# Komputerowe-Projektowanie-Lekow/pmarlo

Hardware: AMD Instinct MI355X
Metric: frames/sec featurize->TICA->k-means->T-matrix, 1Mx64 synth; ITS rel-err (higher is better)
Workload: dtype f64; 1 GPU; synthetic 1000000 frames x 64 f32 features per GPU (AR(1) latents), TICA->10, k=500 (10 Lloyd iterations), lag=10, row-normalised T; frames_per_gpu=1000000, features=64, tica_dim=10, k=500, lag=10, kmeans_iters=10, parallelism=shards1

## Files before the change

### pmarlo_amd/csrc/eig.hip

```cpp
#include "common.h"
#include "wave.h"

__device__ __forceinline__ unsigned long long stamp_clock() {
    unsigned long long t;
    asm volatile("s_memtime %0\n\ts_waitcnt lgkmcnt(0)" : "=s"(t)::"memory");
    return t;
}
#define STAMP_ADD(slot, last) do { const unsigned long long t__ = stamp_clock(); slot += t__ - last; last = t__; } while (0)
#ifdef MSM_JACOBI_STAMPS
__device__ unsigned long long g_jacobi_stamps[8];
#define JSTAMP(i) STAMP_ADD(acc__[i], last__)
#define JSTAMP_INIT unsigned long long acc__[8] = {0, 0, 0, 0, 0, 0, 0, 0}; unsigned long long last__ = stamp_clock();
#define JSTAMP_FLUSH if (threadIdx.x == 0) { for (int i__ = 0; i__ < 8; ++i__) g_jacobi_stamps[i__] += acc__[i__]; }
#else
#define JSTAMP(i)
#define JSTAMP_INIT
#define JSTAMP_FLUSH
#endif
#ifdef MSM_TRI_STAMPS
__device__ unsigned long long g_tri_stamps[24];
#define TSTAMP(i) do { if (threadIdx.x == 0) STAMP_ADD(g_tri_stamps[i], tlast__); } while (0)
#define TSTAMP_INIT unsigned long long tlast__ = 0; if (threadIdx.x == 0) tlast__ = stamp_clock();
#define KSTAMP(i) do { if (threadIdx.x == 0) STAMP_ADD(g_tri_stamps[i], klast__); } while (0)
#define KSTAMP_INIT unsigned long long klast__ = 0; if (threadIdx.x == 0) klast__ = stamp_clock();
#else
#define TSTAMP(i)
#define TSTAMP_INIT
#define KSTAMP(i)
#define KSTAMP_INIT
#endif
#ifdef MSM_TRI_STAMPS_FINE
#define LSTAMP(i) TSTAMP(i)
#define LSTAMP_INIT TSTAMP_INIT
#else
#define LSTAMP(i)
#define LSTAMP_INIT
#endif

namespace {

constexpr int kEigThreads = 1024;
constexpr int kMaxPairs = 128;

struct JacobiShared {
    double2 cs[kMaxPairs];
    int p[kMaxPairs], q[kMaxPairs];
    int reserved[2 * kMaxPairs];
    double2 cs2[2][32];
    int colw2[2][32], roww2[2][32];
    double red[kEigThreads / 64];
    double bc[4];
    int ibc[4];
};

__device__ __forceinline__ double nr_rcp(double x) {
    double r = __builtin_amdgcn_rcp(x);
    r = fma(r, fma(-x, r, 1.0), r);
    r = fma(r, fma(-x, r, 1.0), r);
    return r;
}
__device__ __forceinline__ double nr_rsqrt(double x) {
    double r = __builtin_amdgcn_rsq(x);
    const double h = 0.5 * x;
    r = r * fma(-h * r, r, 1.5);
    r = r * fma(-h * r, r, 1.5);
    return r;
}

__device__ __forceinline__ void jacobi_rotation(double app, double aqq, double apq, double& c, double& s) {
    c = 1.0; s = 0.0;
    if (apq == 0.0) return;
    const double a = 0.5 * (aqq - app);
    const double h2 = fma(a, a, apq * apq);
    if (!(h2 > 1e-300) || !(h2 < 1e300)) return;
    double rh = __builtin_amdgcn_rsq(h2);
    rh = rh * fma(-0.5 * h2 * rh, rh, 1.5);
    const double h = h2 * rh;
    const double den = fabs(a) + h;
    double rd = __builtin_amdgcn_rcp(den);
    rd = fma(rd, fma(-den, rd, 1.0), rd);
    const double t = (a >= 0.0 ? apq : -apq) * rd;
    c = nr_rsqrt(fma(t, t, 1.0));
    s = t * c;
}

__device__ __forceinline__ void pivot_pair(int round, int i, int npad, int& p, int& q) {
    if (i == 0) { p = round; q = npad - 1; return; }
    p = round + i; if (p >= npad - 1) p -= npad - 1;
    q = round - i; if (q < 0) q += npad - 1;
}

__device__ __forceinline__ void rotate_pair(double c, double s, double& xp, double& xq) {
    const double yp = fma(-s, xq, c * xp), yq = fma(s, xp, c * xq);
    xp = yp; xq = yq;
}

__device__ __forceinline__ void rotate_block(double app, double apq, double aqp, double aqq, double ca, double sa,
                                             double cb, double sb, bool diagonal, double& npp, double& npq,
                                             double& nqp, double& nqq) {
    const double rpp = fma(-sa, aqp, ca * app), rpq = fma(-sa, aqq, ca * apq);
    const double rqp = fma(sa, app, ca * aqp), rqq = fma(sa, apq, ca * aqq);
    npp = fma(-sb, rpq, cb * rpp); npq = fma(sb, rpp, cb * rpq);
    nqp = fma(-sb, rqq, cb * rqp); nqq = fma(sb, rqp, cb * rqq);
    if (diagonal) { npq = 0.0; nqp = 0.0; }
}

__device__ __forceinline__ void set_identity(double* V, int n, int ld) {
    for (int i = threadIdx.x; i < n * n; i += blockDim.x) V[(i / n) * ld + (i % n)] = (i / n == i % n) ? 1.0 : 0.0;
}

__device__ __forceinline__ bool jacobi_converged(const double* A, int n, int ld, JacobiShared* sh) {
    double off = 0.0, dia = 0.0;
    for (int i = threadIdx.x; i < n * n; i += blockDim.x) {
        const int r = i / n, c = i - r * n;
        const double v = A[r * ld + c];
        if (r == c) dia = fma(v, v, dia); else off = fma(v, v, off);
    }
    off = block_sum_bcast(off, sh->red, sh->bc);
    dia = block_sum_bcast(dia, sh->red, sh->bc);
    const double tol = (double)n * 2.220446049250313e-16;
    return off <= tol * tol * (dia + off) || off == 0.0;
}

__device__ __forceinline__ int jacobi_eigh_pipelined(double* A, double* V, int n, int ld, JacobiShared* sh,
                                                     int max_sweeps);

__device__ __forceinline__ int jacobi_eigh(double* A, double* V, int n, int ld, JacobiShared* sh, int max_sweeps) {
    const int tid = threadIdx.x, nt = blockDim.x;
    {
        const int mh = n / 2;
        if ((n & 1) == 0 && mh >= 4 && mh <= 32 && mh * mh <= nt && mh * n <= 2 * nt && n * ld < 65536 && nt >= 64)
            return jacobi_eigh_pipelined(A, V, n, ld, sh, max_sweeps);
    }
    set_identity(V, n, ld);
    __syncthreads();
    if (n < 2) return 0;
    const int npad = n + (n & 1);
    const int m = npad / 2;
    int sweep = 0;
    JSTAMP_INIT
    for (; sweep < max_sweeps; ++sweep) {
        JSTAMP(0);
        if (jacobi_converged(A, n, ld, sh)) break;
        JSTAMP(1);
        const bool fast = (m * m <= nt) && (m * n <= 2 * nt);
        const int my_ia = tid / m, my_ib = tid - my_ia * m;
        const bool has_blk = tid < m * m;
        const int v_ib0 = tid / n, v_r0 = tid - v_ib0 * n;
        const int v_ib1 = (tid + nt) / n, v_r1 = (tid + nt) - v_ib1 * n;
        const bool has_v0 = tid < m * n, has_v1 = tid + nt < m * n;
        const int my_ia_c = has_blk ? my_ia : 0, my_ib_c = has_blk ? my_ib : 0;
        const int v_ib0_c = has_v0 ? v_ib0 : 0, v_ib1_c = has_v1 ? v_ib1 : 0;
        const int v_r1_c = has_v1 ? v_r1 : 0;
        for (int round = 0; round < npad - 1; ++round) {
            if (tid < m) {
                const int i = tid;
                int p, q;
                pivot_pair(round, i, npad, p, q);
                double c = 1.0, s = 0.0;
                if (q < n) jacobi_rotation(A[p * ld + p], A[q * ld + q], A[p * ld + q], c, s);
                sh->cs[i] = make_double2(c, s); sh->p[i] = p; sh->q[i] = q;
            }
            JSTAMP(2);
            __syncthreads();
            JSTAMP(3);
            if (fast) {
                int pa, qa, pb, qb, vp0, vq0, vp1, vq1;
                pivot_pair(round, my_ia_c, npad, pa, qa);
                pivot_pair(round, my_ib_c, npad, pb, qb);
                pivot_pair(round, v_ib0_c, npad, vp0, vq0);
                pivot_pair(round, v_ib1_c, npad, vp1, vq1);
                const bool row_real = qa < n, col_real = qb < n, v0 = has_v0 && vq0 < n, v1 = has_v1 && vq1 < n;
                const int qa_c = row_real ? qa : pa, qb_c = col_real ? qb : pb;
                const int vq0_c = vq0 < n ? vq0 : vp0, vq1_c = vq1 < n ? vq1 : vp1;
                const double2 ra = sh->cs[my_ia_c], rb = sh->cs[my_ib_c], r0 = sh->cs[v_ib0_c], r1 = sh->cs[v_ib1_c];
                const double app = A[pa * ld + pb], apq = A[pa * ld + qb_c];
                const double aqp = A[qa_c * ld + pb], aqq = A[qa_c * ld + qb_c];
                double x0p = V[v_r0 * ld + vp0], x0q = V[v_r0 * ld + vq0_c];
                double x1p = V[v_r1_c * ld + vp1], x1q = V[v_r1_c * ld + vq1_c];
                const double ca = row_real ? ra.x : 1.0, sa = row_real ? ra.y : 0.0;
                const double cb = col_real ? rb.x : 1.0, sb = col_real ? rb.y : 0.0;
                double npp, npq, nqp, nqq;
                rotate_block(app, apq, aqp, aqq, ca, sa, cb, sb, my_ia_c == my_ib_c, npp, npq, nqp, nqq);
                rotate_pair(r0.x, r0.y, x0p, x0q);
                rotate_pair(r1.x, r1.y, x1p, x1q);
                if (has_blk) A[pa * ld + pb] = npp;
                if (has_blk && col_real) A[pa * ld + qb] = npq;
                if (has_blk && row_real) A[qa * ld + pb] = nqp;
                if (has_blk && row_real && col_real) A[qa * ld + qb] = nqq;
                if (v0) { V[v_r0 * ld + vp0] = x0p; V[v_r0 * ld + vq0] = x0q; }
                if (v1) { V[v_r1_c * ld + vp1] = x1p; V[v_r1_c * ld + vq1] = x1q; }
                JSTAMP(4);
                JSTAMP(5);
            } else {
                for (int blk = tid; blk < m * m; blk += nt) {
                    const int ia = blk / m, ib = blk - ia * m;
                    const int pa = sh->p[ia], qa = sh->q[ia], pb = sh->p[ib], qb = sh->q[ib];
                    const bool row_real = qa < n, col_real = qb < n;
                    if (!row_real && !col_real) continue;
                    const double ca = sh->cs[ia].x, sa = sh->cs[ia].y, cb = sh->cs[ib].x, sb = sh->cs[ib].y;
                    if (!col_real) {
                        double ap = A[pa * ld + pb], aq = A[qa * ld + pb];
                        rotate_pair(ca, sa, ap, aq);
                        A[pa * ld + pb] = ap; A[qa * ld + pb] = aq;
                        continue;
                    }
                    if (!row_real) {
                        double ap = A[pa * ld + pb], aq = A[pa * ld + qb];
                        rotate_pair(cb, sb, ap, aq);
                        A[pa * ld + pb] = ap; A[pa * ld + qb] = aq;
                        continue;
                    }
                    const double app = A[pa * ld + pb], apq = A[pa * ld + qb];
                    const double aqp = A[qa * ld + pb], aqq = A[qa * ld + qb];
                    double npp, npq, nqp, nqq;
                    rotate_block(app, apq, aqp, aqq, ca, sa, cb, sb, ia == ib, npp, npq, nqp, nqq);
                    A[pa * ld + pb] = npp; A[pa * ld + qb] = npq;
                    A[qa * ld + pb] = nqp; A[qa * ld + qb] = nqq;
                }
                JSTAMP(4);
                for (int e = tid; e < m * n; e += nt) {
                    const int ib = e / n, r = e - ib * n;
                    const int pb = sh->p[ib], qb = sh->q[ib];
                    if (qb >= n) continue;
                    const double cb = sh->cs[ib].x, sb = sh->cs[ib].y;
                    double vp = V[r * ld + pb], vq = V[r * ld + qb];
                    rotate_pair(cb, sb, vp, vq);
                    V[r * ld + pb] = vp; V[r * ld + qb] = vq;
                }
                JSTAMP(5);
            }
            __syncthreads();
            JSTAMP(6);
        }
    }
    JSTAMP_FLUSH
    return sweep;
}

__device__ __forceinline__ int jacobi_eigh_pipelined(double* A, double* V, int n, int ld, JacobiShared* sh,
                                                     int max_sweeps) {
    const int tid = threadIdx.x, nt = blockDim.x;
    set_identity(V, n, ld);
    const int m = n / 2, ring = n - 1;
    auto form_rotations = [&](int round, int buf) {
        int p, q;
        pivot_pair(round, tid, n, p, q);
        double c, s;
        jacobi_rotation(A[p * ld + p], A[q * ld + q], A[p * ld + q], c, s);
        sh->cs2[buf][tid] = make_double2(c, s);
        sh->colw2[buf][tid] = p | (q << 16);
        sh->roww2[buf][tid] = (p * ld) | ((q * ld) << 16);
    };
    auto update_block = [&](int ia, int ib, int buf, bool live) {
        const int wr = sh->roww2[buf][ia], wc = sh->colw2[buf][ib];
        const double2 ra = sh->cs2[buf][ia], rb = sh->cs2[buf][ib];
        double* Ap = A + (wr & 0xffff);
        double* Aq = A + (wr >> 16);
        const int pb = wc & 0xffff, qb = wc >> 16;
        const double app = Ap[pb], apq = Ap[qb], aqp = Aq[pb], aqq = Aq[qb];
        double npp, npq, nqp, nqq;
        rotate_block(app, apq, aqp, aqq, ra.x, ra.y, rb.x, rb.y, ia == ib, npp, npq, nqp, nqq);
        if (live) { Ap[pb] = npp; Ap[qb] = npq; Aq[pb] = nqp; Aq[qb] = nqq; }
    };
    const int my_ia = tid / m, my_ib = tid - my_ia * m;
    const bool priority = (my_ib == my_ia) || (my_ia >= 2 && my_ib == my_ia - 2) || (my_ia == 1 && my_ib == 0) ||
                          (my_ia == m - 1 && my_ib == m - 2);
    const bool has_blk = tid < m * m && !priority;
    const int my_ia_c = tid < m * m ? my_ia : 0, my_ib_c = tid < m * m ? my_ib : 0;
    int pr_ia = 0, pr_ib = 0;
    const bool has_pr = tid < 2 * m;
    if (tid < m) { pr_ia = tid; pr_ib = tid; }
    else if (tid < 2 * m) {
        const int j = tid - m;
        if (j == 0) { pr_ia = 1; pr_ib = 0; }
        else if (j == 1) { pr_ia = 2; pr_ib = 0; }
        else if (j == m - 1) { pr_ia = m - 1; pr_ib = m - 2; }
        else { pr_ia = j + 1; pr_ib = j - 1; }
    }
    const int v_ib0 = tid / n, v_r0 = tid - v_ib0 * n;
    const int v_ib1 = (tid + nt) / n, v_r1 = (tid + nt) - v_ib1 * n;
    const bool has_v0 = tid < m * n, has_v1 = tid + nt < m * n;
    const int v_ib0_c = has_v0 ? v_ib0 : 0, v_ib1_c = has_v1 ? v_ib1 : 0, v_r1_c = has_v1 ? v_r1 : 0;
    __syncthreads();
    int buf = 0, round = 0;
    if (tid < m) form_rotations(0, 0);
    __syncthreads();
    int sweep = 0;
    for (; sweep < max_sweeps; ++sweep) {
        if (jacobi_converged(A, n, ld, sh)) break;
        for (int rr = 0; rr < ring; ++rr) {
            const int next_round = round + 1 == ring ? 0 : round + 1;
            if (tid < 64) {
                update_block(pr_ia, pr_ib, buf, has_pr);
                if (tid < m) form_rotations(next_round, buf ^ 1);
            }
            update_block(my_ia_c, my_ib_c, buf, has_blk);
            {
                const int w0 = sh->colw2[buf][v_ib0_c], w1 = sh->colw2[buf][v_ib1_c];
                const double2 r0 = sh->cs2[buf][v_ib0_c], r1 = sh->cs2[buf][v_ib1_c];
                double* V0 = V + v_r0 * ld;
                double* V1 = V + v_r1_c * ld;
                const int vp0 = w0 & 0xffff, vq0 = w0 >> 16, vp1 = w1 & 0xffff, vq1 = w1 >> 16;
                double x0p = V0[vp0], x0q = V0[vq0], x1p = V1[vp1], x1q = V1[vq1];
                rotate_pair(r0.x, r0.y, x0p, x0q);
                rotate_pair(r1.x, r1.y, x1p, x1q);
                if (has_v0) { V0[vp0] = x0p; V0[vq0] = x0q; }
                if (has_v1) { V1[vp1] = x1p; V1[vq1] = x1q; }
            }
            __syncthreads();
            buf ^= 1;
            round = next_round;
        }
    }
    return sweep;
}

__device__ void sort_desc_abs(const double* ev, int n, int* order) {
    rank_order<true>(n, order, [&](int i) { return fabs(ev[i]); });
    __syncthreads();
}

__device__ void canonical_signs(double* M, int n, int ncols, int ld) {
    for (int j = threadIdx.x; j < ncols; j += blockDim.x) {
        double best = -1.0, sgn = 1.0;
        for (int i = 0; i < n; ++i) {
            const double v = M[i * ld + j];
            if (fabs(v) > best) { best = fabs(v); sgn = v < 0.0 ? -1.0 : 1.0; }
        }
        if (sgn < 0.0)
            for (int i = 0; i < n; ++i) M[i * ld + j] = -M[i * ld + j];
    }
    __syncthreads();
}

__device__ bool cholesky_lower_pair(double* Mp, double* Mq, int n, int ld, JacobiShared* sh) {
    const int tid = threadIdx.x, nt = blockDim.x;
    for (int j = 0; j < n; ++j) {
        if (tid < 2) {
            double* M = tid == 0 ? Mp : Mq;
            const double dj = M[j * ld + j];
            sh->ibc[1 + tid] = dj > 0.0 ? 1 : 0;
            if (dj > 0.0) M[j * ld + j] = sqrt(dj);
        }
        __syncthreads();
        if (!sh->ibc[1] || !sh->ibc[2]) return false;
        const double pjj = Mp[j * ld + j], qjj = Mq[j * ld + j];
        for (int i = j + 1 + tid; i < n; i += nt) {
            Mp[i * ld + j] /= pjj;
            Mq[i * ld + j] /= qjj;
        }
        __syncthreads();
        const int m = n - j - 1;
        for (int e = tid; e < m * m; e += nt) {
            const int a = e / m, b = e - a * m;
            if (b <= a) {
                const int ra = (j + 1 + a) * ld, rb = (j + 1 + b) * ld;
                Mp[ra + j + 1 + b] -= Mp[ra + j] * Mp[rb + j];
                Mq[ra + j + 1 + b] -= Mq[ra + j] * Mq[rb + j];
            }
        }
        __syncthreads();
    }
    return true;
}

__device__ void lower_inverse(const double* G, double* X, int n, int ld) {
    const int tid = threadIdx.x, nt = blockDim.x;
    for (int e = tid; e < n * n; e += nt) {
        const int i = e / n, c = e - i * n;
        X[i * ld + c] = i == c ? 1.0 : 0.0;
    }
    __syncthreads();
    for (int k = 0; k < n; ++k) {
        const double gkk = G[k * ld + k];
        for (int c = tid; c <= k; c += nt) X[k * ld + c] /= gkk;
        __syncthreads();
        const int rows = n - k - 1, cols = k + 1;
        for (int e = tid; e < rows * cols; e += nt) {
            const int a = e / cols, c = e - a * cols;
            const int i = k + 1 + a;
            X[i * ld + c] = fma(-G[i * ld + k], X[k * ld + c], X[i * ld + c]);
        }
        __syncthreads();
    }
}

constexpr int kTriMax = 64;
constexpr int kTriLd = 65;
struct TriShared {
    double2 de[kTriMax + 8];
    double d[kTriMax], e[kTriMax], lam[kTriMax], praw[kTriMax], uq[kTriMax], inv[kTriMax];
    double scale, gl, gu;
    double red[kEigThreads / 64];
    int bad;
    double part[16][kTriMax];
    union {
        double2 vw[8][kTriMax];
        alignas(16) double lv[16][kTriMax];
    };
    double vpub[2][kTriMax];
    double taupub[2];
};

template <bool TA, bool TB>
__device__ __forceinline__ void mfma_mm(double* C, const double* A, const double* B, int rows, int cols, int inner, int ld,
                        const double* bscale = nullptr) {
    const int lane = threadIdx.x & 63, wave = threadIdx.x >> 6, nw = blockDim.x >> 6;
    const int j = lane & 15, g = lane >> 4;
    const int tr = (rows + 15) >> 4, tc = (cols + 15) >> 4;
    for (int t = wave; t < tr * tc; t += nw) {
        const int i0 = (t / tc) * 16, c0 = (t - (t / tc) * tc) * 16;
        const bool aok = i0 + j < rows, bok = c0 + j < cols;
        const int ai = aok ? i0 + j : 0, bj = bok ? c0 + j : 0;
        const double bs = bscale ? bscale[bj] : 1.0;
        const v4f64 acc = mfma_tile_acc(
            inner, g, aok, bok, [&](int k) { return TA ? A[k * ld + ai] : A[ai * ld + k]; },
            [&](int k) { return (TB ? B[bj * ld + k] : B[k * ld + bj]) * bs; });
#pragma unroll
        for (int r = 0; r < 4; ++r) {
            const int row = i0 + g + 4 * r, col = c0 + j;
            if (row < rows && col < cols) C[row * ld + col] = acc[r];
        }
    }
    __syncthreads();
}

__device__ __forceinline__ int sturm_count(const TriShared* ts, int nblocks, double x) {
    double pp = 0.0, p = 1.0;
    unsigned bits = 0, w0 = 0;
    for (int b = 0; b < nblocks; ++b) {
        asm volatile("" ::: "memory");
        double2 r[8];
#pragma unroll
        for (int u = 0; u < 8; ++u) r[u] = ts->de[8 * b + u];
#pragma unroll
        for (int u = 0; u < 8; ++u) {
            const double pn = fma(r[u].x - x, p, -(r[u].y * pp));
            bits = __builtin_amdgcn_alignbit(bits, (unsigned)__double2hiint(pn), 31);
            pp = p;
            p = pn;
        }
        if (b & 1) {
            const int ex = max(__builtin_amdgcn_frexp_exp(p), __builtin_amdgcn_frexp_exp(pp));
            p = ldexp(p, -ex);
            pp = ldexp(pp, -ex);
        }
        if (b == 3) { w0 = bits; bits = 0; }
    }
    if (nblocks <= 4) return __popc(bits ^ (bits >> 1));
    const int r1 = 8 * nblocks - 32;
    return __popc(w0 ^ (w0 >> 1)) + __popc(bits ^ ((bits >> 1) | ((w0 & 1u) << (r1 - 1))));
}

template <typename F>
__device__ __forceinline__ void hh_for_groups(int sub, int k, F&& body) {
#pragma unroll
    for (int g = 0; g < 2; ++g)
        if (sub + 32 * g + 24 > k) body(g);
}
__device__ __forceinline__ void householder_phase(double* A, double* QT, int n, TriShared* ts) {
    static_assert(kEigThreads == 1024, "householder_phase deals the rows of A and Q' over sixteen waves");
    constexpr int ld = kTriLd;
    const int lane = threadIdx.x & 63, wave = __builtin_amdgcn_readfirstlane(threadIdx.x >> 6);
    const bool in = lane < n;
    const bool is_a = wave < 8;
#ifdef MSM_TRI_NOQ
    const bool is_q = false;
#else
    const bool is_q = !is_a;
#endif
    const int sub = wave & 7;
    double* part = ts->part[wave];
    const double* parts = ts->part[is_a ? 0 : 8];
    double2* vw = ts->vw[sub];
    double m[8];
#pragma unroll
    for (int t = 0; t < 8; ++t) {
        const int j = sub + 8 * t;
        m[t] = (in && j < n) ? (is_a ? A[j * ld + lane] : (j == lane ? 1.0 : 0.0)) : 0.0;
    }
    auto q_partial = [&](int c) {
        if (__builtin_amdgcn_readfirstlane(ts->taupub[c & 1] != 0.0)) {
            const double* vp = ts->vpub[c & 1];
            double s0 = 0.0, s1 = 0.0;
            hh_for_groups(sub, c, [&](int g) {
                double v[4];
#pragma unroll
                for (int u = 0; u < 4; ++u) v[u] = vp[sub + 32 * g + 8 * u];
                s0 = fma(m[4 * g], v[0], s0);
                s1 = fma(m[4 * g + 1], v[1], s1);
                s0 = fma(m[4 * g + 2], v[2], s0);
                s1 = fma(m[4 * g + 3], v[3], s1);
            });
            part[lane] = s0 + s1;
        }
    };
    auto sum_parts = [&]() {
        return (((parts[lane] + parts[kTriMax + lane]) + (parts[2 * kTriMax + lane] + parts[3 * kTriMax + lane])) +
                ((parts[4 * kTriMax + lane] + parts[5 * kTriMax + lane]) + (parts[6 * kTriMax + lane] + parts[7 * kTriMax + lane])));
    };
    auto q_finish = [&](int c) {
        const double tau_c = ts->taupub[c & 1];
        if (__builtin_amdgcn_readfirstlane(tau_c != 0.0)) {
            const double* vp = ts->vpub[c & 1];
            const double tu = -tau_c * sum_parts();
            hh_for_groups(sub, c, [&](int g) {
                double v[4];
#pragma unroll
                for (int u = 0; u < 4; ++u) v[u] = vp[sub + 32 * g + 8 * u];
#pragma unroll
                for (int u = 0; u < 4; ++u) m[4 * g + u] = fma(tu, v[u], m[4 * g + u]);
            });
        }
    };
    auto reflector = [&](int c, double& vi, double& tau) {
        const double* rowc = A + c * ld;
        double xi = rowc[in ? lane : 0];
        const double alpha = rowc[c + 1];
        if (wave == 0 && lane == c) ts->d[c] = xi;
        const bool actc = in && lane > c;
        if (!actc) xi = 0.0;
        const double sigma = wave_sum_all(lane > c + 1 ? xi * xi : 0.0);
        const bool nz = sigma != 0.0;
        const double h2 = fma(alpha, alpha, sigma);
        const double rs = nr_rsqrt(nz ? h2 : 1.0);
        const double beta = nz ? -copysign(h2 * rs, alpha) : alpha;
        tau = nz ? (beta - alpha) * -copysign(rs, alpha) : 0.0;
        const double scal = nr_rcp(nz ? alpha - beta : 1.0);
        vi = actc ? (lane == c + 1 ? 1.0 : (nz ? xi * scal : 0.0)) : 0.0;
        if (wave == 0) {
            ts->vpub[c & 1][lane] = vi;
            if (lane == 0) { ts->e[c] = beta; ts->taupub[c & 1] = tau; }
        }
        vw[lane].x = vi;
    };
    LSTAMP_INIT
    double vi = 0.0, tau = 0.0;
    if (is_a && n > 2) reflector(0, vi, tau);
    for (int k = 0; k + 2 < n; ++k) {
        LSTAMP(16);
        const bool act = in && lane > k;
        if (is_a) {
            double s0 = 0.0, s1 = 0.0;
            hh_for_groups(sub, k, [&](int g) {
                double v[4];
#pragma unroll
                for (int u = 0; u < 4; ++u) v[u] = vw[sub + 32 * g + 8 * u].x;
                s0 = fma(m[4 * g], v[0], s0);
                s1 = fma(m[4 * g + 1], v[1], s1);
                s0 = fma(m[4 * g + 2], v[2], s0);
                s1 = fma(m[4 * g + 3], v[3], s1);
            });
            part[lane] = s0 + s1;
            LSTAMP(18);
        } else if (is_q && k > 0) {
            q_finish(k - 1);
        }
        __syncthreads();
        LSTAMP(19);
        double wi = 0.0;
        if (is_a) {
            const double p = sum_parts();
            const double pv = wave_sum_all(act ? p * vi : 0.0);
            const double al = -0.5 * tau * (tau * pv);
            wi = act ? fma(tau, p, al * vi) : 0.0;
            vw[lane].y = wi;
            LSTAMP(20);
#pragma unroll
            for (int t2 = 0; t2 < 8; ++t2)
                if (sub + 8 * t2 == k + 1) {
                    const double2 bk = vw[k + 1];
                    if (in) A[(k + 1) * ld + lane] = fma(-wi, bk.x, fma(-vi, bk.y, m[t2]));
                }
        } else if (is_q) {
            q_partial(k);
        }
        LSTAMP(21);
        __syncthreads();
        if (is_a) {
            double2 bb[8];
#pragma unroll
            for (int t2 = 0; t2 < 8; ++t2) bb[t2] = vw[sub + 8 * t2];
            const double vk = vi, wk = wi;
            if (k + 3 < n) reflector(k + 1, vi, tau);
#pragma unroll
            for (int t2 = 0; t2 < 8; ++t2) m[t2] = fma(-wk, bb[t2].x, fma(-vk, bb[t2].y, m[t2]));
            LSTAMP(17);
        }
    }
    if (is_q && n > 2) q_finish(n - 3);
    if (is_q && in) {
#pragma unroll
        for (int t = 0; t < 8; ++t)
            if (sub + 8 * t < n) QT[(sub + 8 * t) * ld + lane] = m[t];
    }
    if (is_a && in) {
#pragma unroll
        for (int t = 0; t < 8; ++t)
            if (sub + 8 * t >= n - 2 && sub + 8 * t < n) A[(sub + 8 * t) * ld + lane] = m[t];
    }
    __syncthreads();
    if (threadIdx.x == 0) {
        ts->d[n - 2] = A[(n - 2) * ld + n - 2];
        ts->e[n - 2] = A[(n - 1) * ld + n - 2];
        ts->d[n - 1] = A[(n - 1) * ld + n - 1];
        ts->e[n - 1] = 0.0;
    }
}

__device__ __forceinline__ bool ldl_whiten_registers(const double* C, double* W, int n, double epsilon, TriShared* ts,
                                                     int mode) {
    static_assert(kEigThreads == 1024, "ldl_whiten_registers deals the rows over sixteen waves");
    constexpr int ld = kTriLd;
    const int lane = threadIdx.x & 63, wave = __builtin_amdgcn_readfirstlane(threadIdx.x >> 6);
    const bool in = lane < n;
    const int what = mode == 2 ? (wave < 8 ? 2 : 3) : (wave < 8 ? 0 : 1);
    const int src = mode == 2 ? 2 : 0;
    const int sub = wave & 7;
    double m[8];
#pragma unroll
    for (int t = 0; t < 8; ++t) {
        const int i = sub + 8 * t;
        if (what == 1) m[t] = lane == i ? 1.0 : 0.0;
        else m[t] = (what < 3 && in && i < n) ? C[i * ld + lane] - (what == 2 && lane == i ? epsilon : 0.0) : 0.0;
    }
    if (sub == 0 && what < 3) ts->part[what][lane] = m[0];
    __syncthreads();
    LSTAMP_INIT
    for (int j = 0; j < n; ++j) {
        const int par = (j & 1) * 4;
        if (what < 3) {
            const double rowM = ts->part[par + src][lane];
            const double row = what == 1 ? ts->part[par + 1][lane] : rowM;
            const double d = readlane_f64(rowM, j);
            LSTAMP(13);
            if (!(d > 0.0)) return false;
            {
                const double lvec = lane > j ? rowM * nr_rcp(d) : 0.0;
                double* lv = ts->lv[wave];
                lv[(lane & 7) * 8 + (lane >> 3)] = lvec;
                const double2* mine = reinterpret_cast<const double2*>(lv + sub * 8);
#pragma unroll
                for (int t2 = 0; t2 < 4; ++t2) {
                    const double2 l = mine[t2];
                    m[2 * t2] = fma(-l.x, row, m[2 * t2]);
                    m[2 * t2 + 1] = fma(-l.y, row, m[2 * t2 + 1]);
                }
                if (((j + 1 - sub) & 7) == 0) {
                    double* dst = ts->part[(par ^ 4) + what] + lane;
                    switch ((j + 1 - sub) >> 3) {
                        case 0: *dst = m[0]; break;   case 1: *dst = m[1]; break;   case 2: *dst = m[2]; break;
                        case 3: *dst = m[3]; break;   case 4: *dst = m[4]; break;   case 5: *dst = m[5]; break;
                        case 6: *dst = m[6]; break;   case 7: *dst = m[7]; break;   default: break;
                    }
                }
            }
        } else {
            const double dP = ts->part[par + src][j];
            if (!(dP > 0.0)) return false;
        }
        LSTAMP(14);
        __syncthreads();
        LSTAMP(15);
    }
    if (what == 0) {
#pragma unroll
        for (int t = 0; t < 8; ++t)
            if (lane == sub + 8 * t && lane < n) ts->inv[lane] = nr_rsqrt(m[t]);
    }
    __syncthreads();
    if (what == 1 && in) {
#pragma unroll
        for (int t = 0; t < 8; ++t) {
            const int i = sub + 8 * t;
            if (i < n) W[lane * ld + i] = m[t] * ts->inv[i];
        }
    }
    __syncthreads();
    return true;
}

constexpr double kTriGuard = 1e-6;
__device__ __forceinline__ bool tridiag_eigh(double* A, double* Q, double* X, int n, int ld, TriShared* ts, double orth_tol,
                                             int want, int* sel, int& kept) {
    const int tid = threadIdx.x, nt = blockDim.x, lane = tid & 63, wave = tid >> 6;
    kept = 0;
    if (n == 1) {
        if (tid == 0) { ts->lam[0] = A[0]; A[0] = 1.0; }
        __syncthreads();
        return true;
    }
    if (ld != kTriLd) return false;
    TSTAMP_INIT
    if (tid == 0) ts->bad = 0;
    __syncthreads();
    TSTAMP(0);
    householder_phase(A, Q, n, ts);
    TSTAMP(1);
    __syncthreads();
    TSTAMP(2);
    {
        const double dl = lane < n ? ts->d[lane] : 0.0, el = lane < n ? ts->e[lane] : 0.0;
        double an = fmax(fabs(dl), fabs(el));
#pragma unroll
        for (int off = 32; off > 0; off >>= 1) an = fmax(an, __shfl_xor(an, off, 64));
        double sc = 1.0;
        if (an > 0.0 && an < 1e300) { int ex; (void)frexp(an, &ex); sc = ldexp(1.0, -ex); }
        const double ds = dl * sc, es = el * sc;
        const double em = lane > 0 && lane < n ? ts->e[lane - 1] * sc : 0.0;
        const double rad = fabs(em) + (lane + 1 < n ? fabs(es) : 0.0);
        double gl = lane < n ? ds - rad : 1e300, gu = lane < n ? ds + rad : -1e300;
        wave_minmax_xor(gl, gu);
        __syncthreads();
        if (wave == 0) {
            if (lane < n) { ts->d[lane] = ds; ts->e[lane] = es; ts->de[lane] = make_double2(ds, em * em); }
            else ts->de[lane] = make_double2(8.0, 0.0);
            if (lane < 8) ts->de[kTriMax + lane] = make_double2(8.0, 0.0);
            if (lane == 0) {
                if (!(an < 1e300)) ts->bad = 1;
                ts->scale = sc;
                const double bn = fmax(fabs(gl), fabs(gu));
                const double pad = 4.0 * n * 2.220446049250313e-16 * bn + 1e-290;
                ts->gl = gl - pad;
                ts->gu = gu + pad;
            }
        }
    }
    __syncthreads();
    TSTAMP(3);
    if (ts->bad) return false;
    bool lead = want > 0 && 2 * (want + 2) < n;
    int nb = lead ? 2 * (want + 2) : n;
    int na = n;
    for (;;) {
        if (tid < 8 * kTriMax && wave * 8 < nb) {
            const int b = tid >> 3, t = tid & 7;
            const int i = !lead || b < want + 2 ? b : n - nb + b;
            const int nblocks = (n + 7) >> 3;
            double lo = ts->gl, hi = ts->gu;
            const double frac = (double)(t + 1) * (1.0 / 9.0);
            for (int it = 0; it < 20; ++it) {
                const double x = fma(hi - lo, frac, lo);
                const int c = sturm_count(ts, nblocks, x);
                double nlo = c <= i ? x : lo, nhi = c > i ? x : hi;
                lo = row8_reduce(nlo, hw_max_f64);
                hi = row8_reduce(nhi, hw_min_f64);
            }
            if (b < nb && t == 0) ts->lam[i] = 0.5 * (lo + hi);
        }
        __syncthreads();
        if (!lead) break;
        const int nc = 2 * (want + 1);
        const auto cand = [&](int c) { return c <= want ? c : n - nc + c; };
        const auto key = [&](int c) { return fabs(ts->lam[cand(c)] / ts->scale); };
        rank_order<true>(nc, sel, key);
        __syncthreads();
        const bool lone = ts->lam[want + 1] - ts->lam[want] > kTriGuard &&
                          ts->lam[n - want - 1] - ts->lam[n - want - 2] > kTriGuard;
        if (lone && key(sel[want - 1]) != key(sel[want])) {
            const double lk = tid < nc ? ts->lam[cand(tid)] : 0.0;
            __syncthreads();
            if (tid < nc) ts->lam[tid] = lk;
            __syncthreads();
            na = nc;
            break;
        }
        __syncthreads();
        lead = false;
        nb = n;
    }
    TSTAMP(4);
    const double tiny = 1e-290;
    double* Xc = X + (lane < na ? lane : 0);
    double* Ac = A + (lane < na ? lane : 0);
    const double lamb = ts->lam[lane < na ? lane : 0];
    if (wave == 0 && lane < na) {
        double q = ts->de[0].x - lamb;
        Xc[0] = q;
        for (int j0 = 1; j0 < n; j0 += 8) {
            double2 r[8];
#pragma unroll
            for (int u = 0; u < 8; ++u) r[u] = ts->de[j0 + u];
#pragma unroll
            for (int u = 0; u < 8; ++u) {
                if (j0 + u < n) {
                    if (fabs(q) < tiny) q = -tiny;
                    q = fma(-r[u].y, nr_rcp(q), r[u].x - lamb);
                    Xc[(j0 + u) * ld] = q;
                }
            }
        }
    } else if (wave == 1 && lane < na) {
        double r = ts->de[n - 1].x - lamb;
        if (fabs(r) < tiny) r = -tiny;
        double ir = nr_rcp(r);
        Ac[(n - 1) * ld] = ir;
        for (int j0 = n - 2; j0 >= 0; j0 -= 8) {
            double dj[8], e2[8];
#pragma unroll
            for (int u = 0; u < 8; ++u) {
                const int j = j0 - u >= 0 ? j0 - u : 0;
                dj[u] = ts->de[j].x;
                e2[u] = ts->de[j + 1].y;
            }
#pragma unroll
            for (int u = 0; u < 8; ++u) {
                if (j0 - u >= 0) {
                    r = fma(-e2[u], ir, dj[u] - lamb);
                    if (fabs(r) < tiny) r = -tiny;
                    ir = nr_rcp(r);
                    Ac[(j0 - u) * ld] = ir;
                }
            }
        }
    }
    __syncthreads();
    int kk = n - 1;
    if (wave < 2 && lane < na) {
        double gbest = fabs(Xc[(n - 1) * ld]);
        for (int j0 = n - 2; j0 >= 0; j0 -= 8) {
            double g[8];
#pragma unroll
            for (int u = 0; u < 8; ++u) {
                const int j = j0 - u >= 0 ? j0 - u : 0;
                g[u] = fabs(fma(-ts->de[j + 1].y, Ac[(j + 1) * ld], Xc[j * ld]));
            }
#pragma unroll
            for (int u = 0; u < 8; ++u)
                if (j0 - u >= 0 && g[u] <= gbest) { gbest = g[u]; kk = j0 - u; }
        }
    }
    __syncthreads();
    if (wave == 0 && lane < na) {
        double z = 1.0, nrm2 = 1.0;
        for (int j0 = n - 2; j0 >= 0; j0 -= 8) {
            double f[8];
#pragma unroll
            for (int u = 0; u < 8; ++u) {
                const int j = j0 - u >= 0 ? j0 - u : 0;
                double qq = Xc[j * ld];
                if (fabs(qq) < tiny) qq = -tiny;
                f[u] = -(ts->e[j] * nr_rcp(qq));
            }
#pragma unroll
            for (int u = 0; u < 8; ++u) {
                if (j0 - u >= 0 && j0 - u < kk) {
                    z = f[u] * z;
                    Xc[(j0 - u) * ld] = z;
                    nrm2 = fma(z, z, nrm2);
                }
            }
        }
        Xc[kk * ld] = 1.0;
        ts->praw[lane] = nrm2;
    } else if (wave == 1 && lane < na) {
        double z = 1.0, nrm2 = 0.0;
        for (int j0 = 0; j0 + 1 < n; j0 += 8) {
            double f[8];
#pragma unroll
            for (int u = 0; u < 8; ++u) {
                const int j = j0 + u + 1 < n ? j0 + u : 0;
                f[u] = -(ts->e[j] * Ac[(j + 1) * ld]);
            }
#pragma unroll
            for (int u = 0; u < 8; ++u) {
                if (j0 + u + 1 < n && j0 + u >= kk) {
                    z = f[u] * z;
                    Xc[(j0 + u + 1) * ld] = z;
                    nrm2 = fma(z, z, nrm2);
                }
            }
        }
        ts->uq[lane] = nrm2;
    }
    __syncthreads();
    if (tid < na) {
        const double nrm2 = ts->praw[tid] + ts->uq[tid];
        const bool ok = nrm2 > 0.0 && nrm2 < 1e300;
        ts->inv[tid] = nr_rsqrt(ok ? nrm2 : 1.0);
        if (!ok) ts->bad = 1;
    }
    __syncthreads();
    TSTAMP(5);
    {
        double worst = 0.0;
        bool bad = false;
        for (int e0 = tid; e0 < n * na; e0 += nt) {
            const int j = e0 / na, i = e0 - j * na;
            const double x0 = X[j * ld + i];
            const double xm = j > 0 ? ts->e[j - 1] * X[(j - 1) * ld + i] : 0.0;
            const double xp = j + 1 < n ? ts->e[j] * X[(j + 1) * ld + i] : 0.0;
            const double tx = fma(ts->d[j] - ts->lam[i], x0, xm + xp) * ts->inv[i];
            bad = bad || !(fabs(tx) <= 1e-10);
        }
        const int jj = lane & 15, g = lane >> 4;
        const int tiles = (na + 15) >> 4;
        for (int t = wave; t < tiles * tiles; t += nt >> 6) {
            const int a0 = (t / tiles) * 16, b0 = (t - (t / tiles) * tiles) * 16;
            if (b0 > a0) continue;
            const bool aok = a0 + jj < na, bok = b0 + jj < na;
            const int ai = aok ? a0 + jj : 0, bi = bok ? b0 + jj : 0;
            const double sa = ts->inv[ai], sb = ts->inv[bi];
            const v4f64 acc = mfma_tile_acc(
                n, g, aok, bok, [&](int k) { return X[k * ld + ai] * sa; }, [&](int k) { return X[k * ld + bi] * sb; });
#pragma unroll
            for (int r = 0; r < 4; ++r) {
                const int row = a0 + g + 4 * r, col = b0 + jj;
                if (row < na && col < na) worst = fmax(worst, fabs(acc[r] - (row == col ? 1.0 : 0.0)));
            }
        }
        if (bad) worst = 1e300;
#pragma unroll
        for (int off = 32; off > 0; off >>= 1) worst = fmax(worst, __shfl_xor(worst, off, 64));
        if (lane == 0) ts->red[wave] = worst;
        __syncthreads();
        worst = 0.0;
        for (int w = 0; w < nt / 64; ++w) worst = fmax(worst, ts->red[w]);
        TSTAMP(6);
        if (ts->bad || !(worst <= orth_tol)) return false;
    }
    mfma_mm<true, false>(A, Q, X, n, na, n, ld, ts->inv);
    if (tid < na) ts->lam[tid] /= ts->scale;
    __syncthreads();
    TSTAMP(7);
    kept = na < n ? na : 0;
    return true;
}

__device__ __forceinline__ int eigh_with_fallback(double* A, double* V, double* X, int n, int ld, double* backup,
                                                  bool try_tri, TriShared* ts, JacobiShared* sh, double orth_tol,
                                                  double* ev_out, const double*& vec, int want, int& kept) {
    const int tid = threadIdx.x, nt = blockDim.x;
    kept = 0;
    if (try_tri) {
        for (int e = tid; e < n * n; e += nt) backup[e] = A[(e / n) * ld + (e % n)];
        __syncthreads();
        if (tridiag_eigh(A, V, X, n, ld, ts, orth_tol, want, sh->p, kept)) {
            for (int i = tid; i < (kept ? kept : n); i += nt) ev_out[i] = ts->lam[i];
            vec = A;
            return 0;
        }
        kept = 0;
        __syncthreads();
        for (int e = tid; e < n * n; e += nt) A[(e / n) * ld + (e % n)] = backup[e];
        __syncthreads();
    }
    const int sweeps = jacobi_eigh(A, V, n, ld, sh, 40);
    for (int i = tid; i < n; i += nt) ev_out[i] = A[i * ld + i];
    vec = V;
    return sweeps;
}

struct TicaWork {
    double *A, *V, *B1, *B2, *ev, *mean, *isc;
    int* order;
};

template <int lds_mats>
__global__ __launch_bounds__(kEigThreads) void tica_solve_kernel(
    const double* __restrict__ mom, const double* __restrict__ scale, int n, int ld, double epsilon, int kinetic_map,
    int n_lead, TicaWork wk, double* __restrict__ out_eig, double* __restrict__ out_W, double* __restrict__ out_mean,
    int* __restrict__ out_rank) {
    extern __shared__ __attribute__((aligned(16))) unsigned char smem_raw[];
    __shared__ JacobiShared sh;
    __shared__ TriShared ts;
    const int tid = threadIdx.x, nt = blockDim.x;
    double* lds = reinterpret_cast<double*>(smem_raw);
    const size_t mat = (size_t)n * ld;
    double *A, *V, *B1, *B2;
    if constexpr (lds_mats >= 2) { A = lds; V = lds + mat; } else { A = wk.A; V = wk.V; }
    if constexpr (lds_mats >= 4) { B1 = lds + 2 * mat; B2 = lds + 3 * mat; } else { B1 = wk.B1; B2 = wk.B2; }

    const double* M00 = mom;
    const double* M0t = mom + (size_t)n * n;
    const double* sx = M0t + (size_t)n * n;
    const double* sy = sx + n;
    const double T = sy[n];
    const double w = 2.0 * T;
    KSTAMP_INIT
    if (!(T > 0.0)) {
        if (tid == 0) *out_rank = 0;
        for (int i = tid; i < n; i += nt) { out_eig[i] = 0.0; out_mean[i] = 0.0; }
        for (int i = tid; i < n * n; i += nt) out_W[i] = 0.0;
        return;
    }
    double* iscp = (lds_mats == 4 && n <= kTriMax) ? ts.lam : wk.isc;
    double* meanp = (lds_mats == 4 && n <= kTriMax) ? ts.inv : wk.mean;
    for (int i = tid; i < n; i += nt) {
        const double is = scale ? 1.0 / scale[i] : 1.0;
        iscp[i] = is;
        const double m = (sx[i] + sy[i]) / w * is;
        meanp[i] = m;
        out_mean[i] = m;
    }
    __syncthreads();
    auto build_cov = [&]() {
        for (int e = tid; e < n * n; e += nt) {
            const int i = e / n, j = e - i * n;
            const double ss = iscp[i] * iscp[j];
            const double mm = meanp[i] * meanp[j];
            A[i * ld + j] = 0.5 * (M00[e] + M00[j * n + i]) / w * ss - mm;
            B1[i * ld + j] = (M0t[e] + M0t[j * n + i]) / w * ss - mm;
        }
        __syncthreads();
    };
    build_cov();
    KSTAMP(8);

    constexpr bool kFused = lds_mats == 4;
    bool full_rank;
    if (kFused && n <= kTriMax) {
        full_rank = ldl_whiten_registers(A, B2, n, epsilon, &ts, 1);
        if (full_rank) {
            double s = 0.0;
            for (int e = tid; e < n * n; e += nt) {
                const double wv = B2[(e / n) * ld + (e % n)];
                s = fma(wv, wv, s);
            }
            s = block_sum_bcast(s, sh.red, sh.bc);
            if (!(s * epsilon * (1.0 + 1e-9) <= 1.0)) full_rank = ldl_whiten_registers(A, nullptr, n, epsilon, &ts, 2);
        }
    } else {
        for (int e = tid; e < n * n; e += nt) {
            const int i = e / n, j = e - i * n;
            B2[i * ld + j] = A[i * ld + j] - (i == j ? epsilon : 0.0);
            V[i * ld + j] = A[i * ld + j];
        }
        __syncthreads();
        full_rank = cholesky_lower_pair(B2, V, n, ld, &sh);
        if (full_rank) {
            lower_inverse(V, A, n, ld);
            for (int e = tid; e < n * n; e += nt) {
                const int i = e / n, j = e - i * n;
                B2[i * ld + j] = j >= i ? A[j * ld + i] : 0.0;
            }
            __syncthreads();
        } else {
            __syncthreads();
            build_cov();
        }
    }
    KSTAMP(9);
    int rank;
    if (full_rank) {
        rank = n;
        if (tid == 0) *out_rank = n;
    } else {
        jacobi_eigh(A, V, n, ld, &sh, 40);
        for (int i = tid; i < n; i += nt) wk.ev[i] = A[i * ld + i];
        __syncthreads();
        sort_desc_abs(wk.ev, n, wk.order);
        if (tid == 0) {
            double evmin = wk.ev[0];
            for (int i = 1; i < n; ++i) evmin = fmin(evmin, wk.ev[i]);
            double eps = epsilon;
            if (evmin < 0.0) eps = fmax(eps, -evmin + 1e-16);
            int rank = 0;
            for (int i = 0; i < n; ++i) rank += fabs(wk.ev[i]) >= eps;
            sh.ibc[0] = rank;
            *out_rank = rank;
        }
        __syncthreads();
        rank = sh.ibc[0];
        if (rank == 0) {
            for (int i = tid; i < n; i += nt) out_eig[i] = 0.0;
            for (int i = tid; i < n * n; i += nt) out_W[i] = 0.0;
            return;
        }
        for (int e = tid; e < n * rank; e += nt) {
            const int i = e / rank, j = e - i * rank;
            B2[i * ld + j] = V[i * ld + wk.order[j]];
        }
        __syncthreads();
        canonical_signs(B2, n, rank, ld);
        for (int e = tid; e < n * rank; e += nt) {
            const int i = e / rank, j = e - i * rank;
            B2[i * ld + j] /= sqrt(wk.ev[wk.order[j]]);
        }
        __syncthreads();
    }
    mfma_mm<false, false>(A, B1, B2, n, rank, n, ld);
    mfma_mm<true, false>(V, B2, A, rank, rank, n, ld);
    for (int e = tid; e < rank * rank; e += nt) {
        const int i = e / rank, j = e - i * rank;
        A[i * ld + j] = 0.5 * (V[i * ld + j] + V[j * ld + i]);
    }
    __syncthreads();
    KSTAMP(10);
    const int keep = n_lead > 0 && n_lead < rank ? n_lead : rank;
    const bool lds_tail = kFused && n <= kTriMax;
    const double* Vec;
    int kept;
    eigh_with_fallback(A, V, B1, rank, ld, wk.A, kFused && rank <= kTriMax, &ts, &sh, 1e-11, wk.ev, Vec,
                       lds_tail && keep < rank ? keep : 0, kept);
    __syncthreads();
    KSTAMP(11);
    if (lds_tail) {
        double* evl = ts.praw;
        double* sgn = ts.uq;
        int* ord = sh.p;
        const int ncol = kept ? kept : rank;
        if (tid < ncol) evl[tid] = wk.ev[tid];
        __syncthreads();
        rank_order<true>(ncol, ord, [&](int i) { return fabs(evl[i]); });
        mfma_mm<false, false>(B1, B2, Vec, n, ncol, rank, ld);
        {
            const int lane = tid & 63, wave = tid >> 6;
            for (int j = wave; j < ncol; j += nt >> 6) {
                double best = lane < n ? fabs(B1[lane * ld + j]) : -1.0;
                int bi = lane;
                double val = lane < n ? B1[lane * ld + j] : 0.0;
                wave_argmax_xor(best, bi, val);
                if (lane == 0) sgn[j] = val < 0.0 ? -1.0 : 1.0;
            }
        }
        __syncthreads();
        for (int e = tid; e < n * n; e += nt) {
            const int i = e / n, j = e - i * n;
            double v = 0.0;
            if (j < keep) {
                const int c = ord[j];
                v = B1[i * ld + c] * sgn[c];
                if (kinetic_map) v *= evl[c];
            }
            out_W[e] = v;
        }
        for (int j = tid; j < n; j += nt) out_eig[j] = j < keep ? evl[ord[j]] : 0.0;
        KSTAMP(12);
        return;
    }
    sort_desc_abs(wk.ev, rank, wk.order);
    mfma_mm<false, false>(B1, B2, Vec, n, rank, rank, ld);
    canonical_signs(B1, n, rank, ld);
    for (int e = tid; e < n * n; e += nt) {
        const int i = e / n, j = e - i * n;
        double v = 0.0;
        if (j < keep) {
            v = B1[i * ld + wk.order[j]];
            if (kinetic_map) v *= wk.ev[wk.order[j]];
        }
        out_W[e] = v;
    }
    for (int j = tid; j < n; j += nt) out_eig[j] = j < keep ? wk.ev[wk.order[j]] : 0.0;
    KSTAMP(12);
}

template <bool use_lds>
__global__ __launch_bounds__(kEigThreads) void eigh_kernel(const double* __restrict__ Ain, int n, int ld,
                                                          double* gA, double* gV, int* order,
                                                          double* __restrict__ out_w, double* __restrict__ out_v,
                                                          int* __restrict__ out_sweeps) {
    extern __shared__ __attribute__((aligned(16))) unsigned char smem_raw[];
    __shared__ JacobiShared sh;
    __shared__ TriShared ts;
    const int tid = threadIdx.x, nt = blockDim.x;
    double *A, *V;
    if constexpr (use_lds) { A = reinterpret_cast<double*>(smem_raw); V = A + (size_t)n * ld; }
    else { A = gA; V = gV; }
    for (int e = tid; e < n * n; e += nt) {
        const int i = e / n, j = e - i * n;
        A[i * ld + j] = 0.5 * (Ain[e] + Ain[j * n + i]);
    }
    __syncthreads();
    const double* vec;
    int kept;
    const int sweeps = eigh_with_fallback(A, V, V + (size_t)n * ld, n, ld, gA, use_lds && n <= kTriMax, &ts, &sh, 1e-12,
                                          out_w, vec, 0, kept);
    if (vec == A) {
        if (out_v)
            for (int e = tid; e < n * n; e += nt) out_v[e] = A[(e / n) * ld + (e % n)];
        if (tid == 0 && out_sweeps) *out_sweeps = 0;
        return;
    }
    rank_order<false>(n, order, [&](int i) { return A[i * ld + i]; });
    __syncthreads();
    for (int j = tid; j < n; j += nt) out_w[j] = A[order[j] * ld + order[j]];
    if (out_v)
        for (int e = tid; e < n * n; e += nt) {
            const int i = e / n, j = e - i * n;
            out_v[e] = V[i * ld + order[j]];
        }
    if (tid == 0 && out_sweeps) *out_sweeps = sweeps;
}

template <bool use_lds>
__global__ __launch_bounds__(kEigThreads) void onesided_eig_kernel(const double* __restrict__ mom, int n, int ld,
                                                                  double clip, double* gP, double* gbak, double* gw,
                                                                  int* order, double* __restrict__ out_eig) {
    extern __shared__ __attribute__((aligned(16))) unsigned char smem_raw[];
    __shared__ JacobiShared sh;
    __shared__ TriShared ts;
    const int tid = threadIdx.x, nt = blockDim.x;
    const size_t mat = (size_t)n * ld;
    double* P0 = use_lds ? reinterpret_cast<double*>(smem_raw) : gP;
    double *P1 = P0 + mat, *P2 = P0 + 2 * mat, *P3 = P0 + 3 * mat;
    const double* M00 = mom;
    const double* M0t = mom + (size_t)n * n;
    const double* sx = M0t + (size_t)n * n;
    const double* sy = sx + n;
    const double T = sy[n];
    if (!(T > 0.0)) {
        for (int i = tid; i < n; i += nt) out_eig[i] = 0.0;
        return;
    }
    const double den = T - 1.0 > 1.0 ? T - 1.0 : 1.0;
    for (int e = tid; e < n * n; e += nt) {
        const int i = e / n, j = e - i * n;
        const double c0 = 0.5 * (M00[e] + M00[j * n + i]) - sx[i] * sx[j] / T;
        P0[i * ld + j] = c0 / den;
        P1[i * ld + j] = (M0t[e] - sx[i] * sy[j] / T) / den;
    }
    __syncthreads();
    auto eigh = [&](const double*& vec) {
        int kept;
        eigh_with_fallback(P0, P2, P3, n, ld, gbak, use_lds && n <= kTriMax, &ts, &sh, 1e-12, gw, vec, 0, kept);
        __syncthreads();
    };
    const double* vec = nullptr;
    eigh(vec);
    for (int e = tid; e < n * n; e += nt) {
        const int i = e / n, j = e - i * n;
        const double wj = gw[j] > clip ? gw[j] : clip;
        P3[i * ld + j] = vec[i * ld + j] / sqrt(sqrt(wj));
    }
    __syncthreads();
    mfma_mm<false, true>(P0, P3, P3, n, n, n, ld);
    mfma_mm<false, false>(P2, P0, P1, n, n, n, ld);
    mfma_mm<false, false>(P3, P2, P0, n, n, n, ld);
    for (int e = tid; e < n * n; e += nt) {
        const int i = e / n, j = e - i * n;
        P0[i * ld + j] = 0.5 * (P3[i * ld + j] + P3[j * ld + i]);
    }
    __syncthreads();
    eigh(vec);
    rank_order<true>(n, order, [&](int i) { return gw[i]; });
    __syncthreads();
    for (int j = tid; j < n; j += nt) out_eig[j] = gw[order[j]];
}

size_t jacobi_lds_bytes(int n, int ld) { return (size_t)(n <= kTriMax ? 3 : 2) * n * ld * sizeof(double); }

constexpr size_t kLdsPerWorkgroup = 160 * 1024;
constexpr size_t kStaticLdsJacobi = sizeof(JacobiShared);
constexpr size_t kStaticLdsTri = sizeof(JacobiShared) + sizeof(TriShared);
static_assert(sizeof(JacobiShared) == 5808 && sizeof(TriShared) == 21808, "update the sizes restated in tests/_eig_ref.py");
constexpr size_t lds_cap(size_t budget, size_t static_bytes) {
    return budget < kLdsPerWorkgroup - static_bytes ? budget : kLdsPerWorkgroup - static_bytes;
}

int eig_ld(int n) { return n <= kTriMax ? kTriLd : (n | 1); }

template <typename... Params, typename... Args>
msm_status launch_single_workgroup(msm_ctx* ctx, void (*kern)(Params...), size_t lds_bytes, Args... args) {
    if (lds_bytes > 48 * 1024)
        MSM_HIP(ctx, hipFuncSetAttribute((const void*)kern, hipFuncAttributeMaxDynamicSharedMemorySize, (int)lds_bytes));
    hipLaunchKernelGGL(kern, dim3(1), dim3(kEigThreads), lds_bytes, ctx->stream, args...);
    MSM_CHECK_LAUNCH(ctx);
    return MSM_OK;
}

}

extern "C" {

msm_status msm_tica_solve(msm_ctx* ctx, const double* d_moments, const double* d_scale, int F, double epsilon,
                          int kinetic_map, double* d_eigvals, double* d_coeffs, double* d_mean, int* d_rank) {
    return msm_tica_solve_leading(ctx, d_moments, d_scale, F, epsilon, kinetic_map, d_eigvals, d_coeffs, d_mean, d_rank, 0);
}

msm_status msm_tica_solve_leading(msm_ctx* ctx, const double* d_moments, const double* d_scale, int F, double epsilon,
                                  int kinetic_map, double* d_eigvals, double* d_coeffs, double* d_mean, int* d_rank,
                                  int n_lead) {
    if (!ctx) return MSM_ERR_INVALID;
    MSM_REQUIRE(ctx, F >= 1 && F <= 2 * kMaxPairs, "msm_tica_solve: need 1 <= F <= %d (got %d)", 2 * kMaxPairs, F);
    MSM_REQUIRE(ctx, epsilon >= 0.0, "msm_tica_solve: epsilon must be >= 0");
    MSM_REQUIRE(ctx, d_moments && d_eigvals && d_coeffs && d_mean && d_rank, "msm_tica_solve: NULL pointer");
    const int ld = eig_ld(F);
    const size_t mat = (size_t)F * ld;
    const size_t need = (4 * mat + 3 * F) * sizeof(double) + (size_t)F * sizeof(int) + 64;
    msm_status rs = msm_reserve_scratch(ctx, need);
    if (rs != MSM_OK) return rs;
    double* base = (double*)ctx->scratch;
    TicaWork wk;
    wk.A = base; wk.V = base + mat; wk.B1 = base + 2 * mat; wk.B2 = base + 3 * mat;
    wk.ev = base + 4 * mat; wk.mean = wk.ev + F; wk.isc = wk.mean + F; wk.order = (int*)(wk.isc + F);
    const size_t lds_budget = 150 * 1024;
    int lds_mats = 0;
    if (4 * mat * sizeof(double) <= lds_cap(lds_budget, kStaticLdsTri)) lds_mats = 4;
    else if (2 * mat * sizeof(double) <= lds_cap(lds_budget, kStaticLdsJacobi)) lds_mats = 2;
    const size_t lds = (size_t)lds_mats * mat * sizeof(double);
    auto kern = lds_mats == 4 ? tica_solve_kernel<4> : (lds_mats == 2 ? tica_solve_kernel<2> : tica_solve_kernel<0>);
    return launch_single_workgroup(ctx, kern, lds, d_moments, d_scale, F, ld, epsilon, kinetic_map,
                                   n_lead > 0 && n_lead < F ? n_lead : 0, wk, d_eigvals, d_coeffs, d_mean, d_rank);
}

msm_status msm_onesided_tica_eigenvalues(msm_ctx* ctx, const double* d_moments, int F, double clip, double* d_eigvals) {
    if (!ctx) return MSM_ERR_INVALID;
    MSM_REQUIRE(ctx, F >= 1 && F <= 2 * kMaxPairs, "msm_onesided_tica_eigenvalues: need 1 <= F <= %d (got %d)",
                2 * kMaxPairs, F);
    MSM_REQUIRE(ctx, d_moments && d_eigvals && clip > 0.0, "msm_onesided_tica_eigenvalues: bad arguments");
    const int ld = eig_ld(F);
    const size_t mat = (size_t)F * ld;
    const size_t lds = 4 * mat * sizeof(double);
    const bool use_lds = lds <= lds_cap(140 * 1024, kStaticLdsTri);
    msm_status rs = msm_reserve_scratch(ctx, ((use_lds ? 0 : 4 * mat) + (size_t)F * F + F) * sizeof(double) +
                                                 (size_t)F * sizeof(int) + 64);
    if (rs != MSM_OK) return rs;
    double* gP = (double*)ctx->scratch;
    double* gbak = gP + (use_lds ? 0 : 4 * mat);
    double* gw = gbak + (size_t)F * F;
    int* order = (int*)(gw + F);
    auto kern = use_lds ? onesided_eig_kernel<true> : onesided_eig_kernel<false>;
    return launch_single_workgroup(ctx, kern, use_lds ? lds : 0, d_moments, F, ld, clip, gP, gbak, gw, order, d_eigvals);
}

msm_status msm_eigh(msm_ctx* ctx, const double* d_a, int n, double* d_w, double* d_v, int* d_sweeps) {
    if (!ctx) return MSM_ERR_INVALID;
    MSM_REQUIRE(ctx, n >= 1 && n <= 2 * kMaxPairs, "msm_eigh: need 1 <= n <= %d (got %d)", 2 * kMaxPairs, n);
    MSM_REQUIRE(ctx, d_a && d_w, "msm_eigh: NULL pointer");
    const int ld = eig_ld(n);
    const size_t mat = (size_t)n * ld;
    msm_status rs = msm_reserve_scratch(ctx, 2 * mat * sizeof(double) + (size_t)n * sizeof(int) + 64);
    if (rs != MSM_OK) return rs;
    double* gA = (double*)ctx->scratch;
    double* gV = gA + mat;
    int* order = (int*)(gV + mat);
    const size_t lds = jacobi_lds_bytes(n, ld);
    const int use_lds = lds <= lds_cap(140 * 1024, kStaticLdsTri);
    auto kern = use_lds ? eigh_kernel<true> : eigh_kernel<false>;
    return launch_single_workgroup(ctx, kern, use_lds ? lds : 0, d_a, n, ld, gA, gV, order, d_w, d_v, d_sweeps);
}

}
```

Baseline: 713.7 million frames/s.

## Block LDL whitening into 4-column panels with f64 MFMA trailing updates

Rewrites the register LDL whitening so that sixteen waves each own a 16x16 tile and elimination advances four pivots at a time. Each trailing update is done with a 16x16x4 f64 MFMA instead of per-column FMA sweeps. This is meant to cut the number of block-wide barriers by about four and to move the rank-1 update arithmetic onto matrix cores. The cost is more complex indexing and a recomputed 4x4 pivot block in every wave. The slicing of the 16-row tiles for the ping-pong buffers may be fragile.

```diff
diff --git a/pmarlo_amd/csrc/eig.hip b/pmarlo_amd/csrc/eig.hip
--- a/pmarlo_amd/csrc/eig.hip
+++ b/pmarlo_amd/csrc/eig.hip
@@ -611,70 +611,105 @@
 
 __device__ __forceinline__ bool ldl_whiten_registers(const double* C, double* W, int n, double epsilon, TriShared* ts,
                                                      int mode) {
-    static_assert(kEigThreads == 1024, "ldl_whiten_registers deals the rows over sixteen waves");
+    static_assert(kEigThreads == 1024 && kTriMax == 64, "ldl_whiten_registers deals 4 x 4 tiles of 16 x 16 over sixteen waves");
     constexpr int ld = kTriLd;
     const int lane = threadIdx.x & 63, wave = __builtin_amdgcn_readfirstlane(threadIdx.x >> 6);
-    const bool in = lane < n;
-    const int what = mode == 2 ? (wave < 8 ? 2 : 3) : (wave < 8 ? 0 : 1);
-    const int src = mode == 2 ? 2 : 0;
-    const int sub = wave & 7;
-    double m[8];
-#pragma unroll
-    for (int t = 0; t < 8; ++t) {
-        const int i = sub + 8 * t;
-        if (what == 1) m[t] = lane == i ? 1.0 : 0.0;
-        else m[t] = (what < 3 && in && i < n) ? C[i * ld + lane] - (what == 2 && lane == i ? epsilon : 0.0) : 0.0;
-    }
-    if (sub == 0 && what < 3) ts->part[what][lane] = m[0];
+    const int jj = lane & 15, g = lane >> 4;
+    const int I = wave >> 2, J = wave & 3, i0 = 16 * I, c0 = 16 * J;
+    const bool with_x = mode == 1;
+    const bool live = i0 < n && c0 < n;
+    v4f64 ac, ax;
+#pragma unroll
+    for (int r = 0; r < 4; ++r) {
+        const int row = i0 + g + 4 * r, col = c0 + jj;
+        const bool ok = row < n && col < n;
+        const double c = C[ok ? row * ld + col : 0];
+        ac[r] = ok ? c - (mode == 2 && row == col ? epsilon : 0.0) : 0.0;
+        ax[r] = ok && row == col ? 1.0 : 0.0;
+    }
+    if (I == 0) {
+        ts->part[g][c0 + jj] = ac[0];
+        ts->part[4 + g][c0 + jj] = ax[0];
+    }
     __syncthreads();
     LSTAMP_INIT
-    for (int j = 0; j < n; ++j) {
-        const int par = (j & 1) * 4;
-        if (what < 3) {
-            const double rowM = ts->part[par + src][lane];
-            const double row = what == 1 ? ts->part[par + 1][lane] : rowM;
-            const double d = readlane_f64(rowM, j);
+    for (int I0 = 0; I0 < 4; ++I0) {
+#pragma unroll
+        for (int r = 0; r < 4; ++r) {
+            const int j0 = 16 * I0 + 4 * r;
+            if (j0 >= n) break;
+            const double* pc = ts->part[8 * (r & 1)];
+            const double* px = pc + 4 * kTriMax;
+            double2 blk[4][2];
+#pragma unroll
+            for (int c = 0; c < 4; ++c)
+#pragma unroll
+                for (int h = 0; h < 2; ++h) blk[c][h] = *reinterpret_cast<const double2*>(pc + c * kTriMax + j0 + 2 * h);
+            const bool ok1 = j0 + 1 < n, ok2 = j0 + 2 < n, ok3 = j0 + 3 < n;
+            const double d0 = blk[0][0].x;
+            bool bad = !(d0 > 0.0);
+            const double r0 = nr_rcp(d0);
+            const double l10 = blk[0][0].y * r0, l20 = blk[0][1].x * r0, l30 = blk[0][1].y * r0;
+            const double b11 = fma(-l10, blk[0][0].y, blk[1][0].y), b12 = fma(-l10, blk[0][1].x, blk[1][1].x);
+            const double b13 = fma(-l10, blk[0][1].y, blk[1][1].y);
+            const double d1 = ok1 ? b11 : 1.0;
+            bad = bad || !(d1 > 0.0);
+            const double r1 = nr_rcp(d1);
+            const double l21 = b12 * r1, l31 = b13 * r1;
+            const double b22 = fma(-l21, b12, fma(-l20, blk[0][1].x, blk[2][1].x));
+            const double b23 = fma(-l21, b13, fma(-l20, blk[0][1].y, blk[2][1].y));
+            const double d2 = ok2 ? b22 : 1.0;
+            bad = bad || !(d2 > 0.0);
+            const double r2 = nr_rcp(d2);
+            const double l32 = b23 * r2;
+            const double b33 = fma(-l32, b23, fma(-l31, b13, fma(-l30, blk[0][1].y, blk[3][1].y)));
+            const double d3 = ok3 ? b33 : 1.0;
+            bad = bad || !(d3 > 0.0);
+            const double r3 = nr_rcp(d3);
             LSTAMP(13);
-            if (!(d > 0.0)) return false;
-            {
-                const double lvec = lane > j ? rowM * nr_rcp(d) : 0.0;
-                double* lv = ts->lv[wave];
-                lv[(lane & 7) * 8 + (lane >> 3)] = lvec;
-                const double2* mine = reinterpret_cast<const double2*>(lv + sub * 8);
-#pragma unroll
-                for (int t2 = 0; t2 < 4; ++t2) {
-                    const double2 l = mine[t2];
-                    m[2 * t2] = fma(-l.x, row, m[2 * t2]);
-                    m[2 * t2 + 1] = fma(-l.y, row, m[2 * t2 + 1]);
+            if (__builtin_amdgcn_readfirstlane((int)bad)) return false;
+            if (with_x && wave == 0 && lane < 4 && j0 + lane < n)
+                ts->inv[j0 + lane] = nr_rsqrt(lane == 0 ? d0 : (lane == 1 ? d1 : (lane == 2 ? d2 : d3)));
+            auto eliminate = [&](const double* rows, int col, double (&u)[4]) {
+                const double p0 = rows[col], p1 = rows[kTriMax + col], p2 = rows[2 * kTriMax + col], p3 = rows[3 * kTriMax + col];
+                u[0] = p0;
+                u[1] = fma(-l10, u[0], p1);
+                u[2] = fma(-l21, u[1], fma(-l20, u[0], p2));
+                u[3] = fma(-l32, u[2], fma(-l31, u[1], fma(-l30, u[0], p3)));
+            };
+            if (live && I >= I0) {
+                double ua[4];
+                eliminate(pc, i0 + jj, ua);
+                const double mg = g == 0 ? ua[0] * r0 : (g == 1 ? ua[1] * r1 : (g == 2 ? ua[2] * r2 : ua[3] * r3));
+                const double a = i0 + jj > j0 + g ? -mg : 0.0;
+                if (J >= I) {
+                    double ub[4];
+                    eliminate(pc, c0 + jj, ub);
+                    const double b = g == 0 ? ub[0] : (g == 1 ? ub[1] : (g == 2 ? ub[2] : ub[3]));
+                    ac = __builtin_amdgcn_mfma_f64_16x16x4f64(a, b, ac, 0, 0, 0);
                 }
-                if (((j + 1 - sub) & 7) == 0) {
-                    double* dst = ts->part[(par ^ 4) + what] + lane;
-                    switch ((j + 1 - sub) >> 3) {
-                        case 0: *dst = m[0]; break;   case 1: *dst = m[1]; break;   case 2: *dst = m[2]; break;
-                        case 3: *dst = m[3]; break;   case 4: *dst = m[4]; break;   case 5: *dst = m[5]; break;
-                        case 6: *dst = m[6]; break;   case 7: *dst = m[7]; break;   default: break;
-                    }
+                if (with_x && J <= I) {
+                    double ux[4];
+                    eliminate(px, c0 + jj, ux);
+                    const double bx = g == 0 ? ux[0] : (g == 1 ? ux[1] : (g == 2 ? ux[2] : ux[3]));
+                    ax = __builtin_amdgcn_mfma_f64_16x16x4f64(a, bx, ax, 0, 0, 0);
                 }
-            }
-        } else {
-            const double dP = ts->part[par + src][j];
-            if (!(dP > 0.0)) return false;
-        }
-        LSTAMP(14);
-        __syncthreads();
-        LSTAMP(15);
-    }
-    if (what == 0) {
-#pragma unroll
-        for (int t = 0; t < 8; ++t)
-            if (lane == sub + 8 * t && lane < n) ts->inv[lane] = nr_rsqrt(m[t]);
-    }
-    __syncthreads();
-    if (what == 1 && in) {
-#pragma unroll
-        for (int t = 0; t < 8; ++t) {
-            const int i = sub + 8 * t;
-            if (i < n) W[lane * ld + i] = m[t] * ts->inv[i];
+                if (j0 + 4 < n && I == (r < 3 ? I0 : I0 + 1)) {
+                    double* nc = ts->part[8 * ((r + 1) & 1)];
+                    nc[g * kTriMax + c0 + jj] = ac[r < 3 ? r + 1 : 0];
+                    nc[(4 + g) * kTriMax + c0 + jj] = ax[r < 3 ? r + 1 : 0];
+                }
+            }
+            LSTAMP(14);
+            __syncthreads();
+            LSTAMP(15);
+        }
+    }
+    if (with_x && live) {
+#pragma unroll
+        for (int r = 0; r < 4; ++r) {
+            const int row = i0 + g + 4 * r, col = c0 + jj;
+            if (row < n && col < n) W[col * ld + row] = ax[r] * ts->inv[row];
         }
     }
     __syncthreads();
```

New measurement: 721.7 million frames/s (median of 6 runs). 1.01x the previous value.
